# DecodeGenetics/BamQC

Measured on AMD Instinct MI355X. Metric: BAM records/sec (and GB/s vs HBM roofline), 150 bp PE, 1/2/4/8 MI355X, higher is better.
Workload: dtype u8/u32/u64 integer

## Files before the change

### bamqc_amd/csrc/k_prep.hip

```cpp
#include <algorithm>
#include <vector>
#include "kernels_common.h"
#include "prep.h"

#define PR_THREADS 256
#define PR_PER_THREAD 4
#define PR_BLOCK (PR_THREADS * PR_PER_THREAD)

__device__ __forceinline__ uint32_t wave_scan_incl_max(uint32_t v)
{
    v = max(v, (uint32_t)__builtin_amdgcn_update_dpp(0, (int)v, 0x111, 0xF, 0xF, true));
    v = max(v, (uint32_t)__builtin_amdgcn_update_dpp(0, (int)v, 0x112, 0xF, 0xF, true));
    v = max(v, (uint32_t)__builtin_amdgcn_update_dpp(0, (int)v, 0x114, 0xF, 0xF, true));
    v = max(v, (uint32_t)__builtin_amdgcn_update_dpp(0, (int)v, 0x118, 0xF, 0xF, true));
    v = max(v, (uint32_t)__builtin_amdgcn_update_dpp(0, (int)v, 0x142, 0xA, 0xF, false));
    v = max(v, (uint32_t)__builtin_amdgcn_update_dpp(0, (int)v, 0x143, 0xC, 0xF, false));
    return v;
}
__device__ __forceinline__ uint32_t block_scan_excl(uint32_t v, uint32_t* sh, uint32_t* total)
{
    const uint32_t inc = wave_scan_incl(v), w = threadIdx.x >> 6, nw = blockDim.x >> 6;
    block_sync();
    if (lane_id() == WAVE - 1) sh[w] = inc;
    block_sync();
    uint32_t base = 0, tot = 0;
    for (uint32_t k = 0; k < nw; ++k) { const uint32_t x = sh[k]; if (k < w) base += x; tot += x; }
    *total = tot;
    return base + inc - v;
}
__device__ __forceinline__ uint32_t block_scan_excl_max(uint32_t v, uint32_t* sh, uint32_t* total)
{
    const uint32_t inc = wave_scan_incl_max(v), w = threadIdx.x >> 6, nw = blockDim.x >> 6;
    block_sync();
    if (lane_id() == WAVE - 1) sh[w] = inc;
    block_sync();
    uint32_t base = 0, tot = 0;
    for (uint32_t k = 0; k < nw; ++k) { const uint32_t x = sh[k]; if (k < w) base = max(base, x); tot = max(tot, x); }
    *total = tot;
    const uint32_t prev = (uint32_t)__builtin_amdgcn_update_dpp(0, (int)inc, 0x138 , 0xF, 0xF, true);
    return max(base, prev);
}
__device__ __forceinline__ unsigned long long uniform64(unsigned long long v)
{
    return (unsigned long long)__builtin_amdgcn_readfirstlane((uint32_t)v) | (unsigned long long)__builtin_amdgcn_readfirstlane((uint32_t)(v >> 32)) << 32;
}
__device__ __forceinline__ void err_key(ErrRec* e, uint32_t read, uint32_t order)
{
    atomicMin(&e->first_key, ((unsigned long long)read << 3) | order);
}

#define PS_THREADS 1024
#define PS_PER (PR_GROUP / (PS_THREADS / 64))
__global__ __launch_bounds__(PS_THREADS) void k_prep_sizes(PrepArgs a)
{
    __shared__ unsigned long long sh[3 * PR_GROUP];
    if (blockIdx.x == 0 && threadIdx.x == 0) {
        a.err->first_key = BQC_ERRKEY_NONE; a.err->flags = 0; a.err->aux0 = a.err->aux1 = 0;
        a.desc->n_cov_extra = 0;
        if (a.pend_extra_n) *a.pend_extra_n = 0;
        if (a.replay) *a.cursor = *a.cursor_save; else *a.cursor_save = *a.cursor;
    }
    for (uint32_t k = blockIdx.x * PS_THREADS + threadIdx.x; k < a.n_sw; k += gridDim.x * PS_THREADS) a.sw_counts[k] = SwCounts{0, 0, 0, 0};
    const uint32_t nblk = (a.n + PR_BLOCK - 1) / PR_BLOCK, bg0 = blockIdx.x * PR_GROUP, nb = min((uint32_t)PR_GROUP, nblk - bg0);
    const uint32_t w = threadIdx.x >> 6, l = lane_id();
    uint4 vl[PS_PER][4];
    uint2 vc[PS_PER][4];
#pragma unroll
    for (int q = 0; q < PS_PER; ++q) {
        const uint32_t bl = w + (PS_THREADS / 64) * q;
        const unsigned long long i0 = (unsigned long long)(bg0 + bl) * PR_BLOCK;
        const bool whole = bl < nb && i0 + PR_BLOCK <= a.n;
#pragma unroll
        for (int j = 0; j < 4; ++j) {
            vl[q][j] = make_uint4(0, 0, 0, 0); vc[q][j] = make_uint2(0, 0);
            if (whole) { const uint32_t i = (uint32_t)i0 + 256u * j + 4u * l; vl[q][j] = *(const uint4*)(a.l_seq + i); vc[q][j] = *(const uint2*)(a.n_cigar + i); }
        }
    }
#pragma unroll
    for (int q = 0; q < PS_PER; ++q) {
        const uint32_t bl = w + (PS_THREADS / 64) * q;
        const unsigned long long i0 = (unsigned long long)(bg0 + bl) * PR_BLOCK;
        unsigned long long s1 = 0, s2 = 0, s3 = 0;
#pragma unroll
        for (int j = 0; j < 4; ++j) {
            const uint4 v = vl[q][j];
            s1 += (unsigned long long)((v.x + 1) / 2) + (v.y + 1) / 2 + (v.z + 1) / 2 + (v.w + 1) / 2;
            s2 += (unsigned long long)v.x + v.y + v.z + v.w;
            s3 += (vc[q][j].x & 0xFFFFu) + (vc[q][j].x >> 16) + (vc[q][j].y & 0xFFFFu) + (vc[q][j].y >> 16);
        }
        if (bl < nb && i0 + PR_BLOCK > a.n)
            for (unsigned long long i = i0 + l; i < a.n; i += WAVE) { const uint32_t L = a.l_seq[i]; s1 += (L + 1) / 2; s2 += L; s3 += a.n_cigar[i]; }
#pragma unroll
        for (int o = 32; o > 0; o >>= 1) { s1 += __shfl_xor(s1, o); s2 += __shfl_xor(s2, o); s3 += __shfl_xor(s3, o); }
        if (l == 0) { sh[3 * bl] = s1; sh[3 * bl + 1] = s2; sh[3 * bl + 2] = s3; }
    }
    block_sync();
    if (threadIdx.x < 3 * PR_GROUP) {
        const uint32_t bl = threadIdx.x / 3, k = threadIdx.x % 3;
        unsigned long long t = 0;
        for (uint32_t j = 0; j < bl; ++j) t += sh[3 * j + k];
        if (bl < nb) a.blk_sizes[3ull * (bg0 + bl) + k] = t;
        if (bl == PR_GROUP - 1) a.grp_sizes[3ull * blockIdx.x + k] = t + sh[3 * bl + k];
    }
}

struct CigarView {
    uint32_t w[4];
    const uint32_t* cg;
    __device__ __forceinline__ uint32_t at(uint32_t k) const
    {
        if (k < 4u) return k == 0u ? w[0] : k == 1u ? w[1] : k == 2u ? w[2] : w[3];
        return cg[k];
    }
};
__device__ __forceinline__ int triplet_eligible(uint32_t flag, uint32_t mapq, int32_t as, const CigarView& cv, uint32_t ncig)
{
    if (!(flag & 0x1) || !(flag & 0x2) || (flag & 0x4) || (flag & 0x8) || (flag & 0x100)) return 0;
    if (mapq < 60) return 0;
    if (as == BQC_AS_ABSENT || as < 0) return -1;
    if (as < 50) return 0;
    uint32_t clipped = 0;
    for (uint32_t k = 0; k < ncig; ++k) {
        const uint32_t wd = cv.at(k), op = wd & 15u;
        if (op == 4u || op == 5u) clipped += wd >> 4;
    }
    return clipped > 0 ? 0 : 1;
}

struct ReadIn { uint32_t L, nc, flag, lane, mapq; int32_t rid, pos, as; CovEntry ce; };
struct ReadOut { uint32_t flag, cls, tgt1; CovEntry ce; };
__device__ __forceinline__ ReadOut prep_one(const PrepArgs& a, const DevRefs& refs, uint32_t i, const ReadIn& in, uint32_t co, bool offsets_ok,
                                            const CigarView& cv, bool ref_loaded , int32_t target_in )
{
    ReadOut o;
    uint32_t flag = in.flag & (0x0FFFu | BQC_FLAG_MATE_MAIN | BQC_FLAG_NO_QUAL);
    const uint32_t L = in.L, lane = in.lane;
    uint32_t nc = in.nc;
    o.tgt1 = 0;
    if (L > a.max_read_len) err_key(a.err, i, 1);
    else if (lane >= a.n_lanes) err_key(a.err, i, 2);
    if (!offsets_ok) nc = 0;
    const bool fast = !a.no_fast && L <= BQC_FAST_MAXLEN;
    uint32_t nseg = 0;
    CovEntry ce = in.ce;
    if (!(flag & 0x900u)) {
        const bool dup = flag & 0x400u, qcf = flag & 0x200u;
        if (!dup && !qcf) {
            const int e = triplet_eligible(flag, in.mapq, in.as, cv, nc);
            if (e < 0) err_key(a.err, i, 4);
            if (e > 0) {
                const int32_t target = target_in;
                if (target < 0 || !ref_loaded) err_key(a.err, i, 5);
                else { o.tgt1 = (uint32_t)target + 1u; flag |= BQC_FLAG_TRIPLET; }
            }
        }
        if (!(flag & 0xC0u)) err_key(a.err, i, 6);
    }
    if (ce.win != BQC_COV_NONE) {
        flag |= BQC_FLAG_COV;
        const bool rc = flag & 0x10u;
        const bool pending = ce.win == BQC_COV_PENDING;
        const uint32_t pend_idx = ce.off_len;
        const int64_t pos = pending ? 0 : (int64_t)ce.off_len;
        uint32_t cc = 0;
        int64_t run_a = -1, run_z = -1;
        bool first = true;
        ce.off_len = 0;
        auto emit = [&](int64_t lo, int64_t hi) {
            if (pending) {
                if (lo < 0 || lo >= 2 * BQC_VSIZE || lo >= hi) return;
                const uint32_t len = (uint32_t)(hi - lo < 2 * BQC_VSIZE ? hi - lo : 2 * BQC_VSIZE);
                if (first) { a.pend[pend_idx] = PendRun{(uint32_t)lo, len}; first = false; return; }
                const uint32_t k = atomicAdd(a.pend_extra_n, 1u);
                if (k < a.pend_extra_cap) a.pend_extra[k] = PendExtra{pend_idx, (uint32_t)lo, len, 0};
                else atomicOr(&a.err->flags, BQC_DEVERR_INTERNAL);
                return;
            }
            hi = hi < 2 * BQC_VSIZE ? hi : 2 * BQC_VSIZE;
            if (lo < 0 || lo >= hi) return;
            const uint32_t v = (uint32_t)lo | ((uint32_t)(hi - lo) << 16);
            if (first) { ce.off_len = v; first = false; return; }
            const uint32_t k = atomicAdd(&a.desc->n_cov_extra, 1u);
            if (k < a.cov_extra_cap) a.cov_extra[k] = CovExtra{ce.win, v, lane, 0};
            else atomicOr(&a.err->flags, BQC_DEVERR_INTERNAL);
        };
        if (nc == 1u) {
            const uint32_t w = cv.w[0], op = w & 15u, nn = w >> 4;
            if (op == 0u || op == 2u) emit(pos, pos + nn);
        } else {
            for (uint32_t k = 0; k < nc; ++k) {
                const uint32_t w = cv.at(rc ? nc - 1 - k : k), op = w & 15u, nn = w >> 4;
                if (op == 4u) cc += nn;
                if (op == 0u || op == 2u) {
                    const int64_t lo = pos + (int64_t)cc, hi = lo + nn;
                    if (run_z == lo) run_z = hi;
                    else { if (run_a >= 0) emit(run_a, run_z); run_a = lo; run_z = hi; }
                    cc += nn;
                }
            }
            if (run_a >= 0) emit(run_a, run_z);
        }
        if (pending) { if (first) a.pend[pend_idx] = PendRun{0, 0}; ce = CovEntry{BQC_COV_NONE, 0}; }
    } else ce.off_len = 0;
    if (fast && (flag & BQC_FLAG_TRIPLET) && nc > 1 && L >= 3) {
        const uint32_t n0 = cv.w[0] >> 4;
        if (n0 != 0) {
            uint64_t rp = n0;
            int64_t cpos = (int64_t)in.pos + n0;
            for (uint32_t k2 = 1; k2 < nc && rp < L; ++k2) {
                const uint32_t wk = cv.at(k2), op = wk & 15u, nn = wk >> 4;
                if (op == 2u || op == 3u || op == 5u || op == 6u) cpos += nn;
                else if (op == 4u || op == 1u) rp += nn;
                else {
                    const uint64_t ia = rp > 1 ? rp : 1, ib = rp + nn < (uint64_t)L - 1 ? rp + nn : (uint64_t)L - 1;
                    const int64_t posv = cpos - (int64_t)rp;
                    if (ia < ib && posv > INT32_MIN / 2 && posv < INT32_MAX / 2) {
                        a.segs[co + nseg] = TripSeg{i, (int32_t)posv, (uint32_t)ia | ((uint32_t)ib << 8), 0};
                        ++nseg;
                    }
                    rp += nn; cpos += nn;
                }
            }
        }
    }
    o.flag = flag;
    o.ce = ce;
    o.cls = ((fast ? ((flag & 0x40u) ? 0u : 1u) : 2u) << 8) | nseg;
    return o;
}

#ifndef PR_WAVES_PER_EU
#define PR_WAVES_PER_EU 4
#endif
__global__ __launch_bounds__(PR_THREADS) __attribute__((amdgpu_waves_per_eu(PR_WAVES_PER_EU, PR_WAVES_PER_EU))) void k_prep_reads(PrepArgs a, DevRefs refs)
{
    __shared__ uint32_t sh[2 * (PR_THREADS / 64)];
    __shared__ uint32_t red[8];
    __shared__ unsigned long long gsum[3 * (PR_THREADS / 64) + 6];
    const uint32_t i0 = blockIdx.x * PR_BLOCK + 4u * threadIdx.x;
    if (threadIdx.x < 8) red[threadIdx.x] = threadIdx.x == 0 ? 0xFFFFFFFFu : 0u;
    const uint32_t grp = blockIdx.x / PR_GROUP, nblk = gridDim.x;
    unsigned long long grp_before[3] = {0, 0, 0}, grp_more[3] = {0, 0, 0}, in_grp = 0;
    for (uint32_t g = threadIdx.x + 2 * PR_THREADS; g < grp; g += PR_THREADS) {
        const unsigned long long* p = (const unsigned long long*)((const char*)a.grp_sizes + 24u * g);
        for (int k = 0; k < 3; ++k) grp_before[k] += p[k];
    }
    if (threadIdx.x < grp) {
        const unsigned long long* p = (const unsigned long long*)((const char*)a.grp_sizes + 24u * threadIdx.x);
        for (int k = 0; k < 3; ++k) grp_before[k] += p[k];
    }
    if (threadIdx.x + PR_THREADS < grp) {
        const unsigned long long* p = (const unsigned long long*)((const char*)a.grp_sizes + 24u * (threadIdx.x + PR_THREADS));
        for (int k = 0; k < 3; ++k) grp_more[k] = p[k];
    }
    if (threadIdx.x < 6) {
        const bool grp_last = (blockIdx.x + 1) % PR_GROUP == 0 || blockIdx.x + 1 == nblk;
        const unsigned long long* incl_p = grp_last ? a.grp_sizes + 3ull * grp : a.blk_sizes + 3ull * (blockIdx.x + 1);
        in_grp = threadIdx.x < 3 ? a.blk_sizes[3ull * blockIdx.x + threadIdx.x] : incl_p[threadIdx.x - 3];
    }
    auto sum_groups = [&] {
        for (int k = 0; k < 3; ++k) grp_before[k] += grp_more[k];
#pragma unroll
        for (int o = 32; o > 0; o >>= 1)
            for (int k = 0; k < 3; ++k) grp_before[k] += __shfl_xor(grp_before[k], o);
        if (lane_id() == 0) for (int k = 0; k < 3; ++k) gsum[3 * (threadIdx.x >> 6) + k] = grp_before[k];
        if (threadIdx.x < 6) gsum[3 * (PR_THREADS / 64) + threadIdx.x] = in_grp;
    };
    ReadIn in[4];
    const uint32_t nlive = i0 >= a.n ? 0u : min(4u, a.n - i0);
    if ((unsigned long long)(blockIdx.x + 1) * PR_BLOCK <= a.n) {
        const uint4 vl = *(const uint4*)(a.l_seq + i0);
        const uint2 vc = *(const uint2*)(a.n_cigar + i0), vf = *(const uint2*)(a.flag_in + i0);
        const uint32_t vlane = *(const uint32_t*)(a.lane + i0), vmq = *(const uint32_t*)(a.mapq + i0);
        const int4 vr = *(const int4*)(a.rid + i0), vp = *(const int4*)(a.pos + i0), va = *(const int4*)(a.as_ + i0);
        const uint4 c01 = *(const uint4*)(a.cov_in + i0), c23 = *(const uint4*)(a.cov_in + i0 + 2);
        asm volatile("" : "+v"(grp_before[0]), "+v"(grp_before[1]), "+v"(grp_before[2]));
        sum_groups();
        const uint32_t Ls[4] = {vl.x, vl.y, vl.z, vl.w}, ncs[4] = {vc.x & 0xFFFFu, vc.x >> 16, vc.y & 0xFFFFu, vc.y >> 16};
        const uint32_t fs[4] = {vf.x & 0xFFFFu, vf.x >> 16, vf.y & 0xFFFFu, vf.y >> 16};
        const int32_t rs[4] = {vr.x, vr.y, vr.z, vr.w}, ps[4] = {vp.x, vp.y, vp.z, vp.w}, as[4] = {va.x, va.y, va.z, va.w};
        const CovEntry cs[4] = {{c01.x, c01.y}, {c01.z, c01.w}, {c23.x, c23.y}, {c23.z, c23.w}};
#pragma unroll
        for (int j = 0; j < 4; ++j) in[j] = ReadIn{Ls[j], ncs[j], fs[j], (vlane >> (8 * j)) & 0xFFu, (vmq >> (8 * j)) & 0xFFu, rs[j], ps[j], as[j], cs[j]};
    } else {
        sum_groups();
#pragma unroll
        for (int j = 0; j < 4; ++j) {
            in[j] = ReadIn{0, 0, 0x900u, 0, 0, -1, 0, 0, CovEntry{BQC_COV_NONE, 0}};
            if ((uint32_t)j < nlive) { const uint32_t i = i0 + j; in[j] = ReadIn{a.l_seq[i], a.n_cigar[i], a.flag_in[i], a.lane[i], a.mapq[i], a.rid[i], a.pos[i], a.as_[i], a.cov_in[i]}; }
        }
    }
    uint32_t ls[4], lq[4], lc[4], ts = 0, tq = 0, tc = 0;
#pragma unroll
    for (int j = 0; j < 4; ++j) { ls[j] = ts; lq[j] = tq; lc[j] = tc; ts += (in[j].L + 1) / 2; tq += in[j].L; tc += in[j].nc; }
    uint32_t tot;
    const uint32_t xs = block_scan_excl(ts, sh, &tot), xq = block_scan_excl(tq, sh, &tot), xc = block_scan_excl(tc, sh, &tot);
    unsigned long long excl[3], incl[3];
    for (int k = 0; k < 3; ++k) {
        unsigned long long t = 0;
        for (uint32_t w = 0; w < PR_THREADS / 64; ++w) t += gsum[3 * w + k];
        grp_before[k] = uniform64(t); excl[k] = uniform64(gsum[3 * (PR_THREADS / 64) + k]); incl[k] = uniform64(gsum[3 * (PR_THREADS / 64) + 3 + k]);
    }
    unsigned long long base[3];
    if (prep_block_bases(grp_before, excl, incl, base) && threadIdx.x == 0) err_key(a.err, blockIdx.x * PR_BLOCK, 3);
    const unsigned long long bs = base[0] + xs, bq = base[1] + xq, bc = base[2] + xc;
    ReadOut out[4];
    CigarView cv[4];
    bool ref_loaded[4];
    int32_t target[4];
    unsigned long long cos[4];
    bool oks[4];
#pragma unroll
    for (int j = 0; j < 4; ++j) {
        const unsigned long long so = bs + ls[j], qo = bq + lq[j], co = bc + lc[j];
        cos[j] = co;
        oks[j] = so + (in[j].L + 1) / 2 <= 0xFFFFFFFFull && qo + in[j].L <= 0xFFFFFFFFull && co + in[j].nc <= 0xFFFFFFFFull;
        const bool live = (uint32_t)j < nlive && oks[j];
        cv[j].cg = a.cigar + (uint32_t)co;
#pragma unroll
        for (uint32_t k = 0; k < 4u; ++k) cv[j].w[k] = live && k < in[j].nc ? cv[j].cg[k] : 0u;
        const int32_t rid = in[j].rid;
        const bool rid_ok = (uint32_t)j < nlive && rid >= 0 && (uint32_t)rid < refs.n_refs;
        ref_loaded[j] = rid_ok && refs.ref[rid] != nullptr;
        target[j] = rid_ok ? (a.fasta_index ? a.fasta_index[rid] : rid) : -1;
    }
    uint32_t tmax = 0, tmin = 0xFFFFFFFFu, maxfast = 0, maxlong = 0, cnt[4] = {0, 0, 0, 0};
    bool local_bad[4] = {false, false, false, false};
#pragma unroll
    for (int j = 0; j < 4; ++j) {
        out[j] = ReadOut{0x900u, 2u << 8, 0, CovEntry{BQC_COV_NONE, 0}};
        if ((uint32_t)j >= nlive) continue;
        out[j] = prep_one(a, refs, i0 + j, in[j], (uint32_t)cos[j], oks[j], cv[j], ref_loaded[j], target[j]);
        if (out[j].tgt1) { local_bad[j] = out[j].tgt1 < tmax; tmax = max(tmax, out[j].tgt1); tmin = min(tmin, out[j].tgt1); }
        const uint32_t cl = out[j].cls >> 8;
        if (cl == 2u) maxlong = max(maxlong, in[j].L); else maxfast = max(maxfast, in[j].L);
        cnt[cl] += 1; cnt[3] += out[j].cls & 0xFFu;
    }
    if (nlive == 4u) {
        *(uint4*)(a.seq_off + i0) = make_uint4((uint32_t)bs + ls[0], (uint32_t)bs + ls[1], (uint32_t)bs + ls[2], (uint32_t)bs + ls[3]);
        *(uint4*)(a.qual_off + i0) = make_uint4((uint32_t)bq + lq[0], (uint32_t)bq + lq[1], (uint32_t)bq + lq[2], (uint32_t)bq + lq[3]);
        *(uint4*)(a.cigar_off + i0) = make_uint4((uint32_t)bc + lc[0], (uint32_t)bc + lc[1], (uint32_t)bc + lc[2], (uint32_t)bc + lc[3]);
        *(uint2*)(a.flag_out + i0) = make_uint2(out[0].flag | (out[1].flag << 16), out[2].flag | (out[3].flag << 16));
        *(uint2*)(a.cls + i0) = make_uint2(out[0].cls | (out[1].cls << 16), out[2].cls | (out[3].cls << 16));
        *(uint4*)(a.cov_out + i0) = make_uint4(out[0].ce.win, out[0].ce.off_len, out[1].ce.win, out[1].ce.off_len);
        *(uint4*)(a.cov_out + i0 + 2) = make_uint4(out[2].ce.win, out[2].ce.off_len, out[3].ce.win, out[3].ce.off_len);
    } else {
        for (uint32_t j = 0; j < nlive; ++j) {
            const uint32_t i = i0 + j;
            a.seq_off[i] = (uint32_t)bs + ls[j]; a.qual_off[i] = (uint32_t)bq + lq[j]; a.cigar_off[i] = (uint32_t)bc + lc[j];
            a.flag_out[i] = (uint16_t)out[j].flag; a.cls[i] = (uint16_t)out[j].cls; a.cov_out[i] = out[j].ce;
        }
    }
    uint32_t blk_max;
    const uint32_t before = block_scan_excl_max(tmax, sh, &blk_max);
#pragma unroll
    for (int j = 0; j < 4; ++j)
        if (out[j].tgt1 && (local_bad[j] || out[j].tgt1 < before)) err_key(a.err, i0 + j, 5);
    if (tmin != 0xFFFFFFFFu) atomicMin(&red[0], tmin);
    if (maxfast) atomicMax(&red[1], maxfast);
    if (maxlong) atomicMax(&red[2], maxlong);
    if (!a.order) {
#pragma unroll
        for (int k = 0; k < 4; ++k) { const uint32_t v = wave_sum(cnt[k]); if (lane_id() == 0 && v) atomicAdd(&red[4 + k], v); }
    }
    block_sync();
    if (threadIdx.x == 0) {
        a.blk_tgt[2ull * blockIdx.x] = blk_max;
        a.blk_tgt[2ull * blockIdx.x + 1] = red[0];
        a.blk_maxfast[2ull * blockIdx.x] = red[1];
        a.blk_maxfast[2ull * blockIdx.x + 1] = red[2];
    }
    if (!a.order && threadIdx.x < 4 && red[4 + threadIdx.x])
        atomicAdd((uint32_t*)&a.sw_counts[blockIdx.x / (BQC_SW_READS / PR_BLOCK)] + threadIdx.x, red[4 + threadIdx.x]);
}

__device__ __forceinline__ uint32_t read_class(const PrepArgs& a, uint32_t r, uint32_t* nseg)
{
    const uint32_t v = a.cls[r];
    *nseg = v & 0xFFu;
    return v >> 8;
}

__global__ __launch_bounds__(PR_THREADS) void k_build_count(PrepArgs a)
{
    __shared__ uint32_t sh[4 * (PR_THREADS / 64)];
    const SuperWindow sw = a.sws[blockIdx.x];
    uint32_t c[4] = {0, 0, 0, 0};
    for (uint32_t p = threadIdx.x; p < sw.count; p += PR_THREADS) {
        const uint32_t r = a.order ? a.order[sw.begin + p] : sw.begin + p;
        uint32_t ns;
        const uint32_t cl = read_class(a, r, &ns);
        c[cl] += 1;
        c[3] += ns;
    }
    for (int k = 0; k < 4; ++k) c[k] = wave_sum(c[k]);
    if (lane_id() == 0) for (int k = 0; k < 4; ++k) sh[4 * (threadIdx.x >> 6) + k] = c[k];
    block_sync();
    if (threadIdx.x < 4) {
        uint32_t t = 0;
        for (uint32_t w = 0; w < PR_THREADS / 64; ++w) t += sh[4 * w + threadIdx.x];
        ((uint32_t*)&a.sw_counts[blockIdx.x])[threadIdx.x] = t;
    }
}

__global__ __launch_bounds__(1024) void k_build_plan(PrepArgs a)
{
    __shared__ uint32_t sh[2 * 16 + 8];
    __shared__ uint32_t s_fast_w, s_first_bad, s_gmin;
    const uint32_t nblk = (a.n + PR_BLOCK - 1) / PR_BLOCK;
    {
        uint32_t carry = (uint32_t)(*a.cursor + 1);
        uint32_t mf = 0, gmin = 0xFFFFFFFFu;
        if (threadIdx.x == 0) { s_first_bad = 0xFFFFFFFFu; s_gmin = 0xFFFFFFFFu; }
        for (uint32_t b0 = 0; b0 < nblk; b0 += blockDim.x) {
            const uint32_t b = b0 + threadIdx.x;
            const uint32_t mx = b < nblk ? a.blk_tgt[2ull * b] : 0u, mn = b < nblk ? a.blk_tgt[2ull * b + 1] : 0xFFFFFFFFu;
// ... 71 lines not shown
        const uint32_t nq_pad = (nq + rpw - 1) / rpw * rpw;
        const uint32_t seg0 = pb + ng * rpw, slow0 = seg0 + nq_pad;
        for (uint32_t s = s_sw0 + threadIdx.x; s < s_sw1; s += blockDim.x) {
            SwPlan p = a.sw_plan[s];
            p.group_base = pb + (p.group_base - s_g0) * rpw;
            p.seg_base = seg0 + (p.seg_base - s_q0);
            p.slow_base = slow0 + (p.slow_base - s_s0);
            a.sw_plan[s] = p;
        }
        for (uint32_t k = nq + threadIdx.x; k < nq_pad; k += blockDim.x) a.perm[seg0 + k] = 0xFFFFFFFFu;
        const uint32_t n_rc = (ng + groups_cap - 1) / groups_cap, n_sc = (nq_pad + seg_cap - 1) / seg_cap, n_lc = (ns + BQC_CHUNK_READS - 1) / BQC_CHUNK_READS;
        const uint32_t cf = s_cf, cs = s_cs;
        for (uint32_t k = threadIdx.x; k < n_rc; k += blockDim.x) {
            const uint32_t g = min(groups_cap, ng - k * groups_cap);
            if (cf + k < a.chunks_fast_cap) a.chunks_fast[cf + k] = Chunk{pb + k * groups_cap * rpw, g * rpw, lane, g * rpw, 0, 0, 0, 0};
        }
        for (uint32_t k = threadIdx.x; k < n_sc; k += blockDim.x) {
            const uint32_t e = min(seg_cap, nq_pad - k * seg_cap);
            if (cf + n_rc + k < a.chunks_fast_cap) a.chunks_fast[cf + n_rc + k] = Chunk{seg0 + k * seg_cap, e, lane, 0, 0, 0, 0, 0};
        }
        for (uint32_t k = threadIdx.x; k < n_lc; k += blockDim.x) {
            const uint32_t e = min((uint32_t)BQC_CHUNK_READS, ns - k * BQC_CHUNK_READS);
            if (cs + k < a.chunks_slow_cap) a.chunks_slow[cs + k] = Chunk{slow0 + k * BQC_CHUNK_READS, e, lane, 0, 0, 0, 0, 0};
        }
        block_sync();
        if (threadIdx.x == 0) { s_pb = slow0 + ns; s_cf = cf + n_rc + n_sc; s_cs = cs + n_lc; }
        block_sync();
    }
    uint32_t longest = 0;
    for (uint32_t b = threadIdx.x; b < nblk; b += blockDim.x) longest = max(longest, a.blk_maxfast[2ull * b + 1]);
    for (int o = 32; o > 0; o >>= 1) longest = max(longest, (uint32_t)__shfl_xor((int)longest, o));
    if (threadIdx.x == 0) s_longest = 0;
    block_sync();
    if (lane_id() == 0) atomicMax(&s_longest, longest);
    block_sync();
    if (threadIdx.x == 0) {
        if (s_pb > a.perm_cap || s_cf > a.chunks_fast_cap || s_cs > a.chunks_slow_cap) atomicOr(&a.err->flags, BQC_DEVERR_INTERNAL);
        const bool fatal = a.err->first_key != BQC_ERRKEY_NONE || (a.err->flags & BQC_DEVERR_INTERNAL);
        a.desc->fatal = fatal ? 1u : 0u;
        a.desc->n_chunks_fast = fatal ? 0u : min(s_cf, a.chunks_fast_cap);
        a.desc->n_chunks_slow = fatal ? 0u : min(s_cs, a.chunks_slow_cap);
        a.desc->fast_w = fast_w;
        a.desc->n_perm = s_pb;
        a.desc->long_max_len = s_longest;
        if (a.desc->n_cov_extra > a.cov_extra_cap) a.desc->n_cov_extra = a.cov_extra_cap;
        const unsigned long long key = a.err->first_key;
        if (key != BQC_ERRKEY_NONE) {
            const uint32_t i = (uint32_t)(key >> 3), order = (uint32_t)key & 7u;
            if (i < a.n) { a.err->aux0 = order == 1 ? a.l_seq[i] : order == 2 ? a.lane[i] : (uint32_t)a.rid[i]; a.err->aux1 = a.lane[i]; }
        }
    }
}

__device__ __forceinline__ void block_scan_excl4(uint32_t v[4], uint32_t* sh, uint32_t tot[4])
{
    const uint32_t w = threadIdx.x >> 6, nw = blockDim.x >> 6;
    uint32_t inc[4];
#pragma unroll
    for (int k = 0; k < 4; ++k) inc[k] = wave_scan_incl(v[k]);
    block_sync();
    if (lane_id() == WAVE - 1) {
#pragma unroll
        for (int k = 0; k < 4; ++k) sh[4 * w + k] = inc[k];
    }
    block_sync();
#pragma unroll
    for (int k = 0; k < 4; ++k) {
        uint32_t base = 0, t = 0;
        for (uint32_t q = 0; q < nw; ++q) { const uint32_t x = sh[4 * q + k]; if (q < w) base += x; t += x; }
        tot[k] = t;
        v[k] = base + inc[k] - v[k];
    }
}

#define SC_PER (BQC_SW_READS / PR_THREADS)
#define SC_ENT (3 * BQC_SW_READS + 128)
__global__ __launch_bounds__(PR_THREADS) void k_build_scatter(PrepArgs a)
{
    __shared__ uint32_t ent[SC_ENT];
    __shared__ uint32_t sh[4 * (PR_THREADS / 64)];
    const SuperWindow sw = a.sws[blockIdx.x];
    const SwPlan pl = a.sw_plan[blockIdx.x];
    const uint32_t fast_w = a.desc->fast_w, rpw = 64u / fast_w, h0 = (rpw + 1) / 2, h1 = rpw / 2;
    const uint32_t n_ent = pl.n_groups * rpw;
    if (n_ent > SC_ENT) { if (threadIdx.x == 0) atomicOr(&a.err->flags, BQC_DEVERR_INTERNAL); return; }
    for (uint32_t k = threadIdx.x; k < n_ent; k += PR_THREADS) ent[k] = 0xFFFFFFFFu;
    uint32_t r[SC_PER], v[SC_PER];
    const uint32_t p0 = SC_PER * threadIdx.x;
    if (!a.order && p0 + SC_PER <= sw.count && ((sw.begin + p0) & 7u) == 0u) {
        const uint4 x = *(const uint4*)(a.cls + sw.begin + p0), y = *(const uint4*)(a.cls + sw.begin + p0 + 8);
        const uint32_t wd[8] = {x.x, x.y, x.z, x.w, y.x, y.y, y.z, y.w};
#pragma unroll
        for (int k = 0; k < SC_PER; ++k) { r[k] = sw.begin + p0 + k; v[k] = (wd[k >> 1] >> (16 * (k & 1))) & 0xFFFFu; }
    } else {
#pragma unroll
        for (int k = 0; k < SC_PER; ++k) { const uint32_t p = p0 + k; r[k] = p < sw.count ? (a.order ? a.order[sw.begin + p] : sw.begin + p) : 0xFFFFFFFFu; }
#pragma unroll
        for (int k = 0; k < SC_PER; ++k) v[k] = r[k] != 0xFFFFFFFFu ? a.cls[r[k]] : 3u << 8;
    }
    uint32_t c[4] = {0, 0, 0, 0};
#pragma unroll
    for (int k = 0; k < SC_PER; ++k) {
        const uint32_t cl = v[k] >> 8;
        c[0] += cl == 0u; c[1] += cl == 1u; c[2] += cl == 2u; c[3] += cl < 3u ? v[k] & 0xFFu : 0u;
    }
    uint32_t co[SC_PER];
#pragma unroll
    for (int k = 0; k < SC_PER; ++k) co[k] = (v[k] >> 8) < 3u && (v[k] & 0xFFu) ? a.cigar_off[r[k]] : 0u;
    uint32_t tot[4];
    block_scan_excl4(c, sh, tot);
    uint32_t k0 = c[0], k1 = c[1], k2 = c[2], k3 = c[3];
#pragma unroll
    for (int k = 0; k < SC_PER; ++k) {
        const uint32_t cl = v[k] >> 8, ns = v[k] & 0xFFu;
        if (cl == 0u) { ent[(k0 / h0) * rpw + k0 % h0] = r[k]; ++k0; }
        else if (cl == 1u) { ent[(k1 / h1) * rpw + h0 + k1 % h1] = r[k]; ++k1; }
        else if (cl == 2u) a.perm[pl.slow_base + k2++] = r[k];
        if (cl < 3u && ns) { for (uint32_t j = 0; j < ns; ++j) a.perm[pl.seg_base + k3 + j] = BQC_ENTRY_SEG | (co[k] + j); k3 += ns; }
    }
    block_sync();
    for (uint32_t k = threadIdx.x; k < n_ent; k += PR_THREADS) a.perm[pl.group_base + k] = ent[k];
}

extern "C" void bqc_launch_prep(const PrepArgs& a, const DevRefs& refs, hipStream_t s, hipEvent_t after_reads)
{
    if (a.n == 0) return;
    const uint32_t nblk = (a.n + PR_BLOCK - 1) / PR_BLOCK;
    hipLaunchKernelGGL(k_prep_sizes, dim3((nblk + PR_GROUP - 1) / PR_GROUP), dim3(PS_THREADS), 0, s, a);
    hipLaunchKernelGGL(k_prep_reads, dim3(nblk), dim3(PR_THREADS), 0, s, a, refs);
    if (after_reads) (void)hipEventRecord(after_reads, s);
    if (a.order) hipLaunchKernelGGL(k_build_count, dim3(a.n_sw), dim3(PR_THREADS), 0, s, a);
    hipLaunchKernelGGL(k_build_plan, dim3(1), dim3(1024), 0, s, a);
    hipLaunchKernelGGL(k_build_scatter, dim3(a.n_sw), dim3(PR_THREADS), 0, s, a);
}

extern "C" uint32_t bqc_prep_group(void) { return PR_GROUP; }
extern "C" uint32_t bqc_prep_bases(const uint64_t* blk_totals, uint32_t n_blocks, uint64_t* bases)
{
    const uint32_t n_groups = (n_blocks + PR_GROUP - 1) / PR_GROUP;
    std::vector<unsigned long long> blk(3ull * n_blocks), grp(3ull * n_groups);
    for (uint32_t g = 0; g < n_groups; ++g)
        for (int k = 0; k < 3; ++k) {
            unsigned long long t = 0;
            for (uint32_t b = g * PR_GROUP; b < std::min(n_blocks, (g + 1) * PR_GROUP); ++b) { blk[3ull * b + k] = t; t += blk_totals[3ull * b + k]; }
            grp[3ull * g + k] = t;
        }
    uint32_t first_bad = 0xFFFFFFFFu;
    for (uint32_t b = 0; b < n_blocks; ++b) {
        const uint32_t g = b / PR_GROUP;
        const bool grp_last = (b + 1) % PR_GROUP == 0 || b + 1 == n_blocks;
        const unsigned long long* incl = grp_last ? &grp[3ull * g] : &blk[3ull * (b + 1)];
        unsigned long long before[3] = {0, 0, 0}, base[3];
        for (uint32_t g2 = 0; g2 < g; ++g2)
            for (int k = 0; k < 3; ++k) before[k] += grp[3ull * g2 + k];
        if (prep_block_bases(before, &blk[3ull * b], incl, base)) first_bad = std::min(first_bad, b);
        for (int k = 0; k < 3; ++k) bases[3ull * b + k] = base[k];
    }
    return first_bad;
}

__device__ __forceinline__ uint32_t pend_interval(uint32_t pos, uint32_t c0, uint32_t len)
{
    const uint32_t lo = pos + c0;
// ... 28 lines not shown
```

Measured before the change: 4.557 billion.

## Split read prep into a simple fast path and a per-read CIGAR walk slow path

Restructures k_prep_reads so reads with a single CIGAR op and no pending coverage take a lightweight prep_simple path, and only the rest take a serialized per-lane walk that reloads their fields from memory. It merges the three block scans into one multi-value scan, overlaps the group-sum reduction with that scan's barrier, and replaces the shuffle reductions with LDS atomics. It also collects error keys into a single atomicMin per thread, packs class counts into one word, and raises waves_per_eu from 4 to 5. The goal is lower register pressure and fewer barriers and atomics per block. The cost is more code complexity, divergence when walk reads are mixed within a wave, and subtle changes to error ordering and overflow semantics.

```diff
diff --git a/bamqc_amd/csrc/k_prep.hip b/bamqc_amd/csrc/k_prep.hip
--- a/bamqc_amd/csrc/k_prep.hip
+++ b/bamqc_amd/csrc/k_prep.hip
@@ -28,9 +28,33 @@
     *total = tot;
     return base + inc - v;
 }
+struct NothingBetween { __device__ __forceinline__ void operator()() const {} };
+template <int N, int NW = 0, class Between = NothingBetween>
+__device__ __forceinline__ void block_scan_excl_n(uint32_t v[N], uint32_t* sh, uint32_t tot[N], Between between = Between())
+{
+    const uint32_t w = threadIdx.x >> 6, nw = NW ? NW : blockDim.x >> 6;
+    uint32_t inc[N];
+#pragma unroll
+    for (int k = 0; k < N; ++k) inc[k] = wave_scan_incl(v[k]);
+    block_sync();
+    if (lane_id() == WAVE - 1) {
+#pragma unroll
+        for (int k = 0; k < N; ++k) sh[N * w + k] = inc[k];
+    }
+    between();
+    block_sync();
+#pragma unroll
+    for (int k = 0; k < N; ++k) {
+        uint32_t base = 0, t = 0;
+        for (uint32_t q = 0; q < nw; ++q) { const uint32_t x = sh[N * q + k]; if (q < w) base += x; t += x; }
+        tot[k] = t;
+        v[k] = base + inc[k] - v[k];
+    }
+}
+template <int NW = 0>
 __device__ __forceinline__ uint32_t block_scan_excl_max(uint32_t v, uint32_t* sh, uint32_t* total)
 {
-    const uint32_t inc = wave_scan_incl_max(v), w = threadIdx.x >> 6, nw = blockDim.x >> 6;
+    const uint32_t inc = wave_scan_incl_max(v), w = threadIdx.x >> 6, nw = NW ? NW : blockDim.x >> 6;
     block_sync();
     if (lane_id() == WAVE - 1) sh[w] = inc;
     block_sync();
@@ -113,49 +137,84 @@
         return cg[k];
     }
 };
-__device__ __forceinline__ int triplet_eligible(uint32_t flag, uint32_t mapq, int32_t as, const CigarView& cv, uint32_t ncig)
-{
-    if (!(flag & 0x1) || !(flag & 0x2) || (flag & 0x4) || (flag & 0x8) || (flag & 0x100)) return 0;
-    if (mapq < 60) return 0;
-    if (as == BQC_AS_ABSENT || as < 0) return -1;
-    if (as < 50) return 0;
-    uint32_t clipped = 0;
-    for (uint32_t k = 0; k < ncig; ++k) {
-        const uint32_t wd = cv.at(k), op = wd & 15u;
-        if (op == 4u || op == 5u) clipped += wd >> 4;
-    }
-    return clipped > 0 ? 0 : 1;
-}
-
-struct ReadIn { uint32_t L, nc, flag, lane, mapq; int32_t rid, pos, as; CovEntry ce; };
-struct ReadOut { uint32_t flag, cls, tgt1; CovEntry ce; };
-__device__ __forceinline__ ReadOut prep_one(const PrepArgs& a, const DevRefs& refs, uint32_t i, const ReadIn& in, uint32_t co, bool offsets_ok,
-                                            const CigarView& cv, bool ref_loaded , int32_t target_in )
-{
+
+struct ReadIn { uint32_t L, nc, flag, lane, mapq; int32_t as; CovEntry ce; };
+struct ReadOut { uint32_t flag, cls, eo; CovEntry ce; };
+#define PR_EO_NONE 7u
+
+struct Quad {
+    uint32_t L[4], nc[2], flag[2], lane, mapq;
+    int32_t rid[4], as[4];
+    uint32_t cov[8];
+    __device__ __forceinline__ uint32_t ncig(int j) const { return (nc[j >> 1] >> (16 * (j & 1))) & 0xFFFFu; }
+    __device__ __forceinline__ ReadIn read(int j) const
+    {
+        return ReadIn{L[j], ncig(j), (flag[j >> 1] >> (16 * (j & 1))) & 0xFFFFu, (lane >> (8 * j)) & 0xFFu, (mapq >> (8 * j)) & 0xFFu, as[j], CovEntry{cov[2 * j], cov[2 * j + 1]}};
+    }
+};
+
+template <class Clipped>
+__device__ __forceinline__ uint32_t read_checks(const PrepArgs& a, const ReadIn& in, uint32_t tgt1_in , Clipped clipped, uint32_t* eo)
+{
+    uint32_t flag = in.flag & (0x0FFFu | BQC_FLAG_MATE_MAIN | BQC_FLAG_NO_QUAL);
+    uint32_t o = in.L > a.max_read_len ? 1u : in.lane >= a.n_lanes ? 2u : PR_EO_NONE;
+    const bool primary = !(flag & 0x900u);
+    const bool counted = primary && !(flag & 0x600u);
+    const bool mapped_pair = (flag & 0x10Fu) == 0x3u && in.mapq >= 60;
+    const bool as_bad = in.as == BQC_AS_ABSENT || in.as < 0;
+    bool eligible = counted && mapped_pair && !as_bad && in.as >= 50;
+    if (eligible) eligible = !clipped();
+    if (counted && mapped_pair && as_bad) o = min(o, 4u);
+    if (eligible && !tgt1_in) o = min(o, 5u);
+    if (eligible && tgt1_in) flag |= BQC_FLAG_TRIPLET;
+    if (primary && !(flag & 0xC0u)) o = min(o, 6u);
+    *eo = o;
+    return flag;
+}
+__device__ __forceinline__ uint32_t mate_class(const PrepArgs& a, uint32_t flag, uint32_t L)
+{
+    return !a.no_fast && L <= BQC_FAST_MAXLEN ? ((flag & 0x40u) ? 0u : 1u) : 2u;
+}
+
+__device__ __forceinline__ ReadOut prep_simple(const PrepArgs& a, const ReadIn& in, uint32_t w0, uint32_t tgt1_in)
+{
+    const uint32_t op = w0 & 15u, nn = w0 >> 4;
     ReadOut o;
-    uint32_t flag = in.flag & (0x0FFFu | BQC_FLAG_MATE_MAIN | BQC_FLAG_NO_QUAL);
-    const uint32_t L = in.L, lane = in.lane;
-    uint32_t nc = in.nc;
-    o.tgt1 = 0;
-    if (L > a.max_read_len) err_key(a.err, i, 1);
-    else if (lane >= a.n_lanes) err_key(a.err, i, 2);
-    if (!offsets_ok) nc = 0;
-    const bool fast = !a.no_fast && L <= BQC_FAST_MAXLEN;
+    o.flag = read_checks(a, in, tgt1_in, [&] { return (op == 4u || op == 5u) && nn > 0; }, &o.eo);
+    o.ce = CovEntry{in.ce.win, 0};
+    if (in.ce.win != BQC_COV_NONE) {
+        o.flag |= BQC_FLAG_COV;
+        const uint32_t pos = in.ce.off_len;
+        if ((op == 0u || op == 2u) && pos < 2u * BQC_VSIZE) {
+            const uint32_t hi = min(pos + nn, 2u * BQC_VSIZE);
+            if (pos < hi) o.ce.off_len = pos | ((hi - pos) << 16);
+        }
+    }
+    o.cls = mate_class(a, o.flag, in.L) << 8;
+    return o;
+}
+
+__device__ __forceinline__ ReadOut prep_walk(const PrepArgs& a, uint32_t i, uint32_t nc_in, uint32_t co, bool offsets_ok, uint32_t tgt1_in)
+{
+    const ReadIn in{a.l_seq[i], offsets_ok ? nc_in : 0u, a.flag_in[i], a.lane[i], a.mapq[i], a.as_[i], a.cov_in[i]};
+    const int32_t bam_pos = a.pos[i];
+    const uint32_t L = in.L, lane = in.lane, nc = in.nc;
+    CigarView cv;
+    cv.cg = a.cigar + co;
+#pragma unroll
+    for (uint32_t k = 0; k < 4u; ++k) cv.w[k] = k < nc ? cv.cg[k] : 0u;
+    ReadOut o;
+    uint32_t flag = read_checks(a, in, tgt1_in, [&] {
+        uint32_t clipped = 0;
+        for (uint32_t k = 0; k < nc; ++k) {
+            const uint32_t wd = cv.at(k), op = wd & 15u;
+            if (op == 4u || op == 5u) clipped += wd >> 4;
+        }
+        return clipped > 0;
+    }, &o.eo);
+    const uint32_t cl = mate_class(a, flag, L);
     uint32_t nseg = 0;
     CovEntry ce = in.ce;
-    if (!(flag & 0x900u)) {
-        const bool dup = flag & 0x400u, qcf = flag & 0x200u;
-        if (!dup && !qcf) {
-            const int e = triplet_eligible(flag, in.mapq, in.as, cv, nc);
-            if (e < 0) err_key(a.err, i, 4);
-            if (e > 0) {
-                const int32_t target = target_in;
-                if (target < 0 || !ref_loaded) err_key(a.err, i, 5);
-                else { o.tgt1 = (uint32_t)target + 1u; flag |= BQC_FLAG_TRIPLET; }
-            }
-        }
-        if (!(flag & 0xC0u)) err_key(a.err, i, 6);
-    }
     if (ce.win != BQC_COV_NONE) {
         flag |= BQC_FLAG_COV;
         const bool rc = flag & 0x10u;
@@ -202,11 +261,11 @@
         }
         if (pending) { if (first) a.pend[pend_idx] = PendRun{0, 0}; ce = CovEntry{BQC_COV_NONE, 0}; }
     } else ce.off_len = 0;
-    if (fast && (flag & BQC_FLAG_TRIPLET) && nc > 1 && L >= 3) {
+    if (cl != 2u && (flag & BQC_FLAG_TRIPLET) && nc > 1 && L >= 3) {
         const uint32_t n0 = cv.w[0] >> 4;
         if (n0 != 0) {
             uint64_t rp = n0;
-            int64_t cpos = (int64_t)in.pos + n0;
+            int64_t cpos = (int64_t)bam_pos + n0;
             for (uint32_t k2 = 1; k2 < nc && rp < L; ++k2) {
                 const uint32_t wk = cv.at(k2), op = wk & 15u, nn = wk >> 4;
                 if (op == 2u || op == 3u || op == 5u || op == 6u) cpos += nn;
@@ -225,18 +284,19 @@
     }
     o.flag = flag;
     o.ce = ce;
-    o.cls = ((fast ? ((flag & 0x40u) ? 0u : 1u) : 2u) << 8) | nseg;
+    o.cls = (cl << 8) | nseg;
     return o;
 }
+__device__ __forceinline__ uint32_t pick4(const uint32_t v[4], uint32_t j) { return j == 0u ? v[0] : j == 1u ? v[1] : j == 2u ? v[2] : v[3]; }
 
 #ifndef PR_WAVES_PER_EU
-#define PR_WAVES_PER_EU 4
+#define PR_WAVES_PER_EU 5
 #endif
 __global__ __launch_bounds__(PR_THREADS) __attribute__((amdgpu_waves_per_eu(PR_WAVES_PER_EU, PR_WAVES_PER_EU))) void k_prep_reads(PrepArgs a, DevRefs refs)
 {
-    __shared__ uint32_t sh[2 * (PR_THREADS / 64)];
+    __shared__ uint32_t sh[3 * (PR_THREADS / 64)];
     __shared__ uint32_t red[8];
-    __shared__ unsigned long long gsum[3 * (PR_THREADS / 64) + 6];
+    __shared__ unsigned long long gsum[3 * (PR_THREADS / 64) + 6], gtot[3];
     const uint32_t i0 = blockIdx.x * PR_BLOCK + 4u * threadIdx.x;
     if (threadIdx.x < 8) red[threadIdx.x] = threadIdx.x == 0 ? 0xFFFFFFFFu : 0u;
     const uint32_t grp = blockIdx.x / PR_GROUP, nblk = gridDim.x;
@@ -259,109 +319,152 @@
         in_grp = threadIdx.x < 3 ? a.blk_sizes[3ull * blockIdx.x + threadIdx.x] : incl_p[threadIdx.x - 3];
     }
     auto sum_groups = [&] {
-        for (int k = 0; k < 3; ++k) grp_before[k] += grp_more[k];
-#pragma unroll
-        for (int o = 32; o > 0; o >>= 1)
-            for (int k = 0; k < 3; ++k) grp_before[k] += __shfl_xor(grp_before[k], o);
-        if (lane_id() == 0) for (int k = 0; k < 3; ++k) gsum[3 * (threadIdx.x >> 6) + k] = grp_before[k];
+        unsigned long long* mine = gsum + 3 * (threadIdx.x >> 6);
+        if (lane_id() == 0) for (int k = 0; k < 3; ++k) mine[k] = 0;
+        if (threadIdx.x < grp) for (int k = 0; k < 3; ++k) atomicAdd(mine + k, grp_before[k] + grp_more[k]);
         if (threadIdx.x < 6) gsum[3 * (PR_THREADS / 64) + threadIdx.x] = in_grp;
     };
-    ReadIn in[4];
+    Quad q;
     const uint32_t nlive = i0 >= a.n ? 0u : min(4u, a.n - i0);
     if ((unsigned long long)(blockIdx.x + 1) * PR_BLOCK <= a.n) {
         const uint4 vl = *(const uint4*)(a.l_seq + i0);
         const uint2 vc = *(const uint2*)(a.n_cigar + i0), vf = *(const uint2*)(a.flag_in + i0);
         const uint32_t vlane = *(const uint32_t*)(a.lane + i0), vmq = *(const uint32_t*)(a.mapq + i0);
-        const int4 vr = *(const int4*)(a.rid + i0), vp = *(const int4*)(a.pos + i0), va = *(const int4*)(a.as_ + i0);
+        const int4 vr = *(const int4*)(a.rid + i0), va = *(const int4*)(a.as_ + i0);
         const uint4 c01 = *(const uint4*)(a.cov_in + i0), c23 = *(const uint4*)(a.cov_in + i0 + 2);
         asm volatile("" : "+v"(grp_before[0]), "+v"(grp_before[1]), "+v"(grp_before[2]));
         sum_groups();
-        const uint32_t Ls[4] = {vl.x, vl.y, vl.z, vl.w}, ncs[4] = {vc.x & 0xFFFFu, vc.x >> 16, vc.y & 0xFFFFu, vc.y >> 16};
-        const uint32_t fs[4] = {vf.x & 0xFFFFu, vf.x >> 16, vf.y & 0xFFFFu, vf.y >> 16};
-        const int32_t rs[4] = {vr.x, vr.y, vr.z, vr.w}, ps[4] = {vp.x, vp.y, vp.z, vp.w}, as[4] = {va.x, va.y, va.z, va.w};
-        const CovEntry cs[4] = {{c01.x, c01.y}, {c01.z, c01.w}, {c23.x, c23.y}, {c23.z, c23.w}};
-#pragma unroll
-        for (int j = 0; j < 4; ++j) in[j] = ReadIn{Ls[j], ncs[j], fs[j], (vlane >> (8 * j)) & 0xFFu, (vmq >> (8 * j)) & 0xFFu, rs[j], ps[j], as[j], cs[j]};
+        q = Quad{{vl.x, vl.y, vl.z, vl.w}, {vc.x, vc.y}, {vf.x, vf.y}, vlane, vmq, {vr.x, vr.y, vr.z, vr.w}, {va.x, va.y, va.z, va.w},
+                 {c01.x, c01.y, c01.z, c01.w, c23.x, c23.y, c23.z, c23.w}};
     } else {
         sum_groups();
-#pragma unroll
-        for (int j = 0; j < 4; ++j) {
-            in[j] = ReadIn{0, 0, 0x900u, 0, 0, -1, 0, 0, CovEntry{BQC_COV_NONE, 0}};
-            if ((uint32_t)j < nlive) { const uint32_t i = i0 + j; in[j] = ReadIn{a.l_seq[i], a.n_cigar[i], a.flag_in[i], a.lane[i], a.mapq[i], a.rid[i], a.pos[i], a.as_[i], a.cov_in[i]}; }
-        }
-    }
-    uint32_t ls[4], lq[4], lc[4], ts = 0, tq = 0, tc = 0;
-#pragma unroll
-    for (int j = 0; j < 4; ++j) { ls[j] = ts; lq[j] = tq; lc[j] = tc; ts += (in[j].L + 1) / 2; tq += in[j].L; tc += in[j].nc; }
-    uint32_t tot;
-    const uint32_t xs = block_scan_excl(ts, sh, &tot), xq = block_scan_excl(tq, sh, &tot), xc = block_scan_excl(tc, sh, &tot);
+        q = Quad{{0, 0, 0, 0}, {0, 0}, {0x09000900u, 0x09000900u}, 0, 0, {-1, -1, -1, -1}, {0, 0, 0, 0}, {BQC_COV_NONE, 0, BQC_COV_NONE, 0, BQC_COV_NONE, 0, BQC_COV_NONE, 0}};
+#pragma unroll
+        for (int j = 0; j < 4; ++j)
+            if ((uint32_t)j < nlive) {
+                const uint32_t i = i0 + j, h = 16 * (j & 1);
+                const CovEntry ce = a.cov_in[i];
+                q.L[j] = a.l_seq[i]; q.rid[j] = a.rid[i]; q.as[j] = a.as_[i]; q.cov[2 * j] = ce.win; q.cov[2 * j + 1] = ce.off_len;
+                q.nc[j >> 1] |= (uint32_t)a.n_cigar[i] << h; q.flag[j >> 1] = (q.flag[j >> 1] & ~(0xFFFFu << h)) | ((uint32_t)a.flag_in[i] << h);
+                q.lane |= (uint32_t)a.lane[i] << (8 * j); q.mapq |= (uint32_t)a.mapq[i] << (8 * j);
+            }
+    }
+    uint32_t ls[4], lq[4], lc[4], x[3] = {0, 0, 0}, tot[3];
+#pragma unroll
+    for (int j = 0; j < 4; ++j) { ls[j] = x[0]; lq[j] = x[1]; lc[j] = x[2]; x[0] += (q.L[j] + 1) / 2; x[1] += q.L[j]; x[2] += q.ncig(j); }
+    block_scan_excl_n<3, PR_THREADS / 64>(x, sh, tot, [&] {
+        if (threadIdx.x < 3) {
+            unsigned long long t = 0;
+            for (uint32_t w = 0; w < PR_THREADS / 64; ++w) t += gsum[3 * w + threadIdx.x];
+            gtot[threadIdx.x] = t;
+        }
+    });
     unsigned long long excl[3], incl[3];
     for (int k = 0; k < 3; ++k) {
-        unsigned long long t = 0;
-        for (uint32_t w = 0; w < PR_THREADS / 64; ++w) t += gsum[3 * w + k];
-        grp_before[k] = uniform64(t); excl[k] = uniform64(gsum[3 * (PR_THREADS / 64) + k]); incl[k] = uniform64(gsum[3 * (PR_THREADS / 64) + 3 + k]);
+        grp_before[k] = uniform64(gtot[k]); excl[k] = uniform64(gsum[3 * (PR_THREADS / 64) + k]); incl[k] = uniform64(gsum[3 * (PR_THREADS / 64) + 3 + k]);
     }
     unsigned long long base[3];
-    if (prep_block_bases(grp_before, excl, incl, base) && threadIdx.x == 0) err_key(a.err, blockIdx.x * PR_BLOCK, 3);
-    const unsigned long long bs = base[0] + xs, bq = base[1] + xq, bc = base[2] + xc;
-    ReadOut out[4];
-    CigarView cv[4];
-    bool ref_loaded[4];
+    const bool over = prep_block_bases(grp_before, excl, incl, base);
+    if (over && threadIdx.x == 0) err_key(a.err, blockIdx.x * PR_BLOCK, 3);
+    const uint32_t bs = (uint32_t)base[0] + x[0], bq = (uint32_t)base[1] + x[1], bc = (uint32_t)base[2] + x[2];
+    uint32_t bad = 0;
+    if (over) {
+#pragma unroll
+        for (int j = 0; j < 4; ++j) {
+            const unsigned long long so = base[0] + x[0] + ls[j], qo = base[1] + x[1] + lq[j], co = base[2] + x[2] + lc[j];
+            if (so + (q.L[j] + 1) / 2 > 0xFFFFFFFFull || qo + q.L[j] > 0xFFFFFFFFull || co + q.ncig(j) > 0xFFFFFFFFull) bad |= 1u << j;
+        }
+        bad &= (1u << nlive) - 1u;
+    }
+    const uint32_t cos[4] = {bc + lc[0], bc + lc[1], bc + lc[2], bc + lc[3]};
+    if (nlive == 4u) {
+        *(uint4*)(a.seq_off + i0) = make_uint4(bs + ls[0], bs + ls[1], bs + ls[2], bs + ls[3]);
+        *(uint4*)(a.qual_off + i0) = make_uint4(bq + lq[0], bq + lq[1], bq + lq[2], bq + lq[3]);
+        *(uint4*)(a.cigar_off + i0) = make_uint4(cos[0], cos[1], cos[2], cos[3]);
+    } else {
+#pragma unroll
+        for (int j = 0; j < 4; ++j)
+            if ((uint32_t)j < nlive) { a.seq_off[i0 + j] = bs + ls[j]; a.qual_off[i0 + j] = bq + lq[j]; a.cigar_off[i0 + j] = cos[j]; }
+    }
+    uint32_t w0[4], tgt1[4], walk = 0, maxfast = 0, maxlong = 0;
+    const uint8_t* ref_ptr[4];
     int32_t target[4];
-    unsigned long long cos[4];
-    bool oks[4];
 #pragma unroll
     for (int j = 0; j < 4; ++j) {
-        const unsigned long long so = bs + ls[j], qo = bq + lq[j], co = bc + lc[j];
-        cos[j] = co;
-        oks[j] = so + (in[j].L + 1) / 2 <= 0xFFFFFFFFull && qo + in[j].L <= 0xFFFFFFFFull && co + in[j].nc <= 0xFFFFFFFFull;
-        const bool live = (uint32_t)j < nlive && oks[j];
-        cv[j].cg = a.cigar + (uint32_t)co;
-#pragma unroll
-        for (uint32_t k = 0; k < 4u; ++k) cv[j].w[k] = live && k < in[j].nc ? cv[j].cg[k] : 0u;
-        const int32_t rid = in[j].rid;
-        const bool rid_ok = (uint32_t)j < nlive && rid >= 0 && (uint32_t)rid < refs.n_refs;
-        ref_loaded[j] = rid_ok && refs.ref[rid] != nullptr;
-        target[j] = rid_ok ? (a.fasta_index ? a.fasta_index[rid] : rid) : -1;
-    }
-    uint32_t tmax = 0, tmin = 0xFFFFFFFFu, maxfast = 0, maxlong = 0, cnt[4] = {0, 0, 0, 0};
+        const bool live = (uint32_t)j < nlive, ok = !((bad >> j) & 1u);
+        const uint32_t nc = q.ncig(j), L = q.L[j];
+        if (live && (!ok || nc > 1u || q.cov[2 * j] == BQC_COV_PENDING)) walk |= 1u << j;
+        w0[j] = live && ok && nc ? a.cigar[cos[j]] : 0u;
+        const int32_t rid = q.rid[j];
+        const bool rid_ok = live && rid >= 0 && (uint32_t)rid < refs.n_refs;
+        ref_ptr[j] = rid_ok ? refs.ref[rid] : nullptr;
+        target[j] = rid_ok ? rid : -1;
+        const bool fast = !a.no_fast && L <= BQC_FAST_MAXLEN;
+        maxfast = max(maxfast, live && fast ? L : 0u); maxlong = max(maxlong, live && !fast ? L : 0u);
+    }
+    if (a.fasta_index) {
+#pragma unroll
+        for (int j = 0; j < 4; ++j) if (target[j] >= 0) target[j] = a.fasta_index[target[j]];
+    }
+    asm volatile("" : "+v"(target[0]), "+v"(target[1]), "+v"(target[2]), "+v"(target[3]), "+v"(ref_ptr[0]), "+v"(ref_ptr[1]), "+v"(ref_ptr[2]), "+v"(ref_ptr[3]));
+#pragma unroll
+    for (int j = 0; j < 4; ++j) tgt1[j] = ref_ptr[j] != nullptr && target[j] >= 0 ? (uint32_t)target[j] + 1u : 0u;
+    uint32_t fc[4];
+    uint32_t ekey = 0xFFFFFFFFu;
+    {
+        ReadOut out[4];
+#pragma unroll
+        for (int j = 0; j < 4; ++j) {
+            out[j] = ReadOut{0x900u, 2u << 8, PR_EO_NONE, CovEntry{BQC_COV_NONE, 0}};
+            if ((uint32_t)j < nlive && !((walk >> j) & 1u)) out[j] = prep_simple(a, q.read(j), w0[j], tgt1[j]);
+            fc[j] = out[j].flag | (out[j].cls << 16);
+            if (out[j].eo != PR_EO_NONE) ekey = min(ekey, (uint32_t)j << 3 | out[j].eo);
+        }
+        if (nlive == 4u) {
+            *(uint2*)(a.flag_out + i0) = make_uint2((fc[0] & 0xFFFFu) | (fc[1] << 16), (fc[2] & 0xFFFFu) | (fc[3] << 16));
+            *(uint2*)(a.cls + i0) = make_uint2((fc[0] >> 16) | (fc[1] & 0xFFFF0000u), (fc[2] >> 16) | (fc[3] & 0xFFFF0000u));
+            *(uint4*)(a.cov_out + i0) = make_uint4(out[0].ce.win, out[0].ce.off_len, out[1].ce.win, out[1].ce.off_len);
+            *(uint4*)(a.cov_out + i0 + 2) = make_uint4(out[2].ce.win, out[2].ce.off_len, out[3].ce.win, out[3].ce.off_len);
+        } else {
+#pragma unroll
+            for (int j = 0; j < 4; ++j)
+                if ((uint32_t)j < nlive) { a.flag_out[i0 + j] = (uint16_t)fc[j]; a.cls[i0 + j] = (uint16_t)(fc[j] >> 16); a.cov_out[i0 + j] = out[j].ce; }
+        }
+    }
+#pragma nounroll
+    for (uint32_t m = walk; m; m &= m - 1u) {
+        const uint32_t jj = (uint32_t)__ffs((int)m) - 1u, i = i0 + jj;
+        const uint32_t nc = ((jj & 2u ? q.nc[1] : q.nc[0]) >> (16u * (jj & 1u))) & 0xFFFFu;
+        const ReadOut r = prep_walk(a, i, nc, pick4(cos, jj), !((bad >> jj) & 1u), pick4(tgt1, jj));
+        a.flag_out[i] = (uint16_t)r.flag; a.cls[i] = (uint16_t)r.cls; a.cov_out[i] = r.ce;
+#pragma unroll
+        for (uint32_t j = 0; j < 4u; ++j) if (jj == j) fc[j] = r.flag | (r.cls << 16);
+        if (r.eo != PR_EO_NONE) ekey = min(ekey, jj << 3 | r.eo);
+    }
+    uint32_t tmax = 0, tmin = 0xFFFFFFFFu, cnt = 0, nseg = 0;
     bool local_bad[4] = {false, false, false, false};
 #pragma unroll
     for (int j = 0; j < 4; ++j) {
-        out[j] = ReadOut{0x900u, 2u << 8, 0, CovEntry{BQC_COV_NONE, 0}};
+        if (!(fc[j] & BQC_FLAG_TRIPLET)) tgt1[j] = 0;
         if ((uint32_t)j >= nlive) continue;
-        out[j] = prep_one(a, refs, i0 + j, in[j], (uint32_t)cos[j], oks[j], cv[j], ref_loaded[j], target[j]);
-        if (out[j].tgt1) { local_bad[j] = out[j].tgt1 < tmax; tmax = max(tmax, out[j].tgt1); tmin = min(tmin, out[j].tgt1); }
-        const uint32_t cl = out[j].cls >> 8;
-        if (cl == 2u) maxlong = max(maxlong, in[j].L); else maxfast = max(maxfast, in[j].L);
-        cnt[cl] += 1; cnt[3] += out[j].cls & 0xFFu;
-    }
-    if (nlive == 4u) {
-        *(uint4*)(a.seq_off + i0) = make_uint4((uint32_t)bs + ls[0], (uint32_t)bs + ls[1], (uint32_t)bs + ls[2], (uint32_t)bs + ls[3]);
-        *(uint4*)(a.qual_off + i0) = make_uint4((uint32_t)bq + lq[0], (uint32_t)bq + lq[1], (uint32_t)bq + lq[2], (uint32_t)bq + lq[3]);
-        *(uint4*)(a.cigar_off + i0) = make_uint4((uint32_t)bc + lc[0], (uint32_t)bc + lc[1], (uint32_t)bc + lc[2], (uint32_t)bc + lc[3]);
-        *(uint2*)(a.flag_out + i0) = make_uint2(out[0].flag | (out[1].flag << 16), out[2].flag | (out[3].flag << 16));
-        *(uint2*)(a.cls + i0) = make_uint2(out[0].cls | (out[1].cls << 16), out[2].cls | (out[3].cls << 16));
-        *(uint4*)(a.cov_out + i0) = make_uint4(out[0].ce.win, out[0].ce.off_len, out[1].ce.win, out[1].ce.off_len);
-        *(uint4*)(a.cov_out + i0 + 2) = make_uint4(out[2].ce.win, out[2].ce.off_len, out[3].ce.win, out[3].ce.off_len);
-    } else {
-        for (uint32_t j = 0; j < nlive; ++j) {
-            const uint32_t i = i0 + j;
-            a.seq_off[i] = (uint32_t)bs + ls[j]; a.qual_off[i] = (uint32_t)bq + lq[j]; a.cigar_off[i] = (uint32_t)bc + lc[j];
-            a.flag_out[i] = (uint16_t)out[j].flag; a.cls[i] = (uint16_t)out[j].cls; a.cov_out[i] = out[j].ce;
-        }
+        if (tgt1[j]) { local_bad[j] = tgt1[j] < tmax; tmax = max(tmax, tgt1[j]); tmin = min(tmin, tgt1[j]); }
+        cnt += 1u << (9u * (fc[j] >> 24)); nseg += (fc[j] >> 16) & 0xFFu;
     }
     uint32_t blk_max;
-    const uint32_t before = block_scan_excl_max(tmax, sh, &blk_max);
+    const uint32_t before = block_scan_excl_max<PR_THREADS / 64>(tmax, sh, &blk_max);
 #pragma unroll
     for (int j = 0; j < 4; ++j)
-        if (out[j].tgt1 && (local_bad[j] || out[j].tgt1 < before)) err_key(a.err, i0 + j, 5);
+        if (tgt1[j] && (local_bad[j] || tgt1[j] < before)) ekey = min(ekey, (uint32_t)j << 3 | 5u);
+    if (ekey != 0xFFFFFFFFu) err_key(a.err, i0 + (ekey >> 3), ekey & 7u);
     if (tmin != 0xFFFFFFFFu) atomicMin(&red[0], tmin);
     if (maxfast) atomicMax(&red[1], maxfast);
     if (maxlong) atomicMax(&red[2], maxlong);
     if (!a.order) {
-#pragma unroll
-        for (int k = 0; k < 4; ++k) { const uint32_t v = wave_sum(cnt[k]); if (lane_id() == 0 && v) atomicAdd(&red[4 + k], v); }
+        const uint32_t c = wave_scan_incl(cnt), sg = wave_scan_incl(nseg);
+        if (lane_id() == WAVE - 1) {
+            for (uint32_t k = 0; k < 3u; ++k) { const uint32_t v = (c >> (9u * k)) & 0x1FFu; if (v) atomicAdd(&red[4 + k], v); }
+            if (sg) atomicAdd(&red[7], sg);
+        }
     }
     block_sync();
     if (threadIdx.x == 0) {
@@ -539,27 +642,6 @@
     }
 }
 
-__device__ __forceinline__ void block_scan_excl4(uint32_t v[4], uint32_t* sh, uint32_t tot[4])
-{
-    const uint32_t w = threadIdx.x >> 6, nw = blockDim.x >> 6;
-    uint32_t inc[4];
-#pragma unroll
-    for (int k = 0; k < 4; ++k) inc[k] = wave_scan_incl(v[k]);
-    block_sync();
-    if (lane_id() == WAVE - 1) {
-#pragma unroll
-        for (int k = 0; k < 4; ++k) sh[4 * w + k] = inc[k];
-    }
-    block_sync();
-#pragma unroll
-    for (int k = 0; k < 4; ++k) {
-        uint32_t base = 0, t = 0;
-        for (uint32_t q = 0; q < nw; ++q) { const uint32_t x = sh[4 * q + k]; if (q < w) base += x; t += x; }
-        tot[k] = t;
-        v[k] = base + inc[k] - v[k];
-    }
-}
-
 #define SC_PER (BQC_SW_READS / PR_THREADS)
 #define SC_ENT (3 * BQC_SW_READS + 128)
 __global__ __launch_bounds__(PR_THREADS) void k_build_scatter(PrepArgs a)
@@ -595,7 +677,7 @@
 #pragma unroll
     for (int k = 0; k < SC_PER; ++k) co[k] = (v[k] >> 8) < 3u && (v[k] & 0xFFu) ? a.cigar_off[r[k]] : 0u;
     uint32_t tot[4];
-    block_scan_excl4(c, sh, tot);
+    block_scan_excl_n<4>(c, sh, tot);
     uint32_t k0 = c[0], k1 = c[1], k2 = c[2], k3 = c[3];
 #pragma unroll
     for (int k = 0; k < SC_PER; ++k) {
```

New measurement: 4.736 billion (median of 6 runs). 3.9% higher.
